# automl/RoBO

Hardware: NVIDIA H100
Metric: EI evals/sec (GP N=4096, D=16, fp64) (higher is better)
Workload: dtype f64

## Files before the change

### robo_b200/csrc/gpk_api.cu

```cuda
#include <algorithm>
#include <climits>
#include <cmath>
#include <cstdarg>
#include <cstdio>
#include <cstring>
#include <cstdlib>
#include <dlfcn.h>
#include <string>
#include <vector>

#include "gpk_gemm.cuh"
#include "gpk_kernels.cuh"
#include "gpk_diag16.cuh"
#include "gpk_ozaki.cuh"
#include "gpk_de.cuh"
#include "gpk_lbfgs.cuh"
#include "gpk_cmaes.cuh"
#include "gpk_direct.cuh"
#include "gpk_es.cuh"
#include "gpk_esmc.cuh"
#include "gpk_rs.cuh"
#include "gpk_hyper.cuh"
#include "gpk_blr.cuh"
#include "gpk_rf.cuh"
// ... 293 lines not shown
    cfg.dynamicSmemBytes = smem;
    cfg.stream = stream;
    cudaLaunchAttribute attr[1];
    attr[0].id = cudaLaunchAttributeClusterDimension;
    attr[0].val.clusterDim.x = (unsigned)cs;
    attr[0].val.clusterDim.y = 1;
    attr[0].val.clusterDim.z = 1;
    cfg.attrs = attr;
    cfg.numAttrs = cs > 1 ? 1 : 0;
    return cudaLaunchKernelEx(&cfg, kernel, KArgs(args)...);
}

int oz_max_clusters(gpk_handle* h, int cs, int* out) {
    if (h->oz_max_clusters[cs] == 0) {
        if (cs == 1) {
            h->oz_max_clusters[cs] = std::max(h->n_sm, 1);
        } else {
            cudaLaunchConfig_t cfg;
            memset(&cfg, 0, sizeof(cfg));
            cfg.gridDim = dim3((unsigned)cs);
            cfg.blockDim = dim3(OZ_THREADS);
            cfg.dynamicSmemBytes = OZ_SMEM;
            cudaLaunchAttribute attr[1];
            attr[0].id = cudaLaunchAttributeClusterDimension;
            attr[0].val.clusterDim.x = (unsigned)cs;
            attr[0].val.clusterDim.y = 1;
            attr[0].val.clusterDim.z = 1;
            cfg.attrs = attr;
            cfg.numAttrs = 1;
            int n = 0;
            CK(cudaOccupancyMaxActiveClusters(&n, gpk_oz_vargemm_kernel, &cfg));
            if (n < 1) { set_err(h, "no cluster of %d int8 contraction CTAs fits on this device", cs); return GPK_CUDA_ERROR; }
            h->oz_max_clusters[cs] = n;
        }
    }
    *out = h->oz_max_clusters[cs];
    return GPK_OK;
}

int launch_oz_contraction(gpk_handle* h, const CUtensorMap& mapP, const CUtensorMap& mapK, int nb, long rows_padded,
                          long NP, long rows, const int* eP, int eK, double* part_ssq, long ldpart) {
    OzArgs o;
    o.nb = nb; o.ncb = (int)(rows_padded / OZ_TN); o.NP = (int)NP; o.rows = (int)rows;
    const int cs = h->oz_cluster;
    o.group = (int)std::min<long>(512, std::max<long>(4, ((long)24 << 20) / ((long)OZ_TN * NP * OZ_S))) / cs * cs;
    o.eP = eP; o.eK = eK;
    o.part_ssq = part_ssq; o.ldpart = ldpart;
    const int persist = h->oz_persist == 3 ? (nb <= 32 ? 1 : 0) : h->oz_persist;
    const int tiles = o.nb * o.ncb;
    int grid = tiles;
    if (persist == 1) {
        int nclusters = 0, rc;
        if ((rc = oz_max_clusters(h, cs, &nclusters))) return rc;
        if (h->oz_grid > 0) nclusters = std::min(nclusters, h->oz_grid);
        grid = cs * std::min(tiles / cs, nclusters);
    }
    h->oz_last_variant = 1 + (persist == 1 ? 8 : 0) + (cs == 2 ? 16 : cs == 4 ? 32 : 0);
    CK(launch_oz(gpk_oz_vargemm_kernel, (unsigned)grid, cs, (size_t)OZ_SMEM, h->stream, mapP, mapK, o));
    CKL();
    return GPK_OK;
}

template <int EPI, int MI = 8>
int launch_gemm(gpk_handle* h, const CUtensorMap& mA, const CUtensorMap& mB, const GemmArgs& a, int njobs,
                cudaStream_t stream = nullptr) {
    static_assert(MI == 8 || (MI == 2 && EPI == EPI_STORE), "128-row tiles, or 32-row chain tiles that store");
    if (njobs <= 0) return GPK_OK;
    if (stream == nullptr) stream = h->stream;
    if constexpr (MI == 2) {
        CK(launch_pdl(gpk_gemm_nt_kernel, dim3(njobs), dim3(GEMM_THREADS), (size_t)GEMM_SMEM_CHAIN, stream, mA, mB, a));
        h->launches_total += 1;
        return GPK_OK;
    }
    gpk_gemm_ws_kernel<EPI><<<njobs, WS_THREADS, GEMM_SMEM_TMA, stream>>>(mA, mB, a);
    CKL();
    return GPK_OK;
}

int set_kernel_attrs(gpk_handle* h) {
    CK(cudaFuncSetAttribute(gpk_gemm_ws_kernel<EPI_STORE>, cudaFuncAttributeMaxDynamicSharedMemorySize, GEMM_SMEM_TMA));
    CK(cudaFuncSetAttribute(gpk_gemm_ws_kernel<EPI_COLREDUCE>, cudaFuncAttributeMaxDynamicSharedMemorySize, GEMM_SMEM_TMA));
    CK(cudaFuncSetAttribute(gpk_gemm_nt_kernel, cudaFuncAttributeMaxDynamicSharedMemorySize, GEMM_SMEM_CHAIN));
    CK(cudaFuncSetAttribute(gpk_oz_vargemm_kernel, cudaFuncAttributeMaxDynamicSharedMemorySize, OZ_SMEM));
    CK(cudaFuncSetAttribute(gpk_cov_oz_kernel<8>, cudaFuncAttributeMaxDynamicSharedMemorySize, (int)cov_oz_smem_bytes(GPK_MAX_TERMS, 8)));
    CK(cudaFuncSetAttribute(gpk_cov_oz_kernel<4>, cudaFuncAttributeMaxDynamicSharedMemorySize, (int)cov_oz_smem_bytes(GPK_MAX_TERMS, 4)));
    CK(cudaFuncSetAttribute(gpk_cov_oz_kernel<8, false>, cudaFuncAttributeMaxDynamicSharedMemorySize, (int)cov_oz_smem_bytes(GPK_MAX_TERMS, 8)));
    {
        cudaDeviceProp prop;
        CK(cudaGetDeviceProperties(&prop, h->device));
        h->n_sm = prop.multiProcessorCount;
    }
    CK(cudaFuncSetAttribute(gpk_cov_tma_kernel<8>, cudaFuncAttributeMaxDynamicSharedMemorySize, (int)cov_tma_smem_bytes(GPK_MAX_TERMS, 8)));
    CK(cudaFuncSetAttribute(gpk_cov_tma_kernel<4>, cudaFuncAttributeMaxDynamicSharedMemorySize, (int)cov_tma_smem_bytes(GPK_MAX_TERMS, 4)));
    CK(cudaFuncSetAttribute(gpk_potrf_diag_dmma_kernel, cudaFuncAttributeMaxDynamicSharedMemorySize, DIAG_SMEM));
    return GPK_OK;
}

struct Node { int lo, mid, hi, height; };

int build_nodes(int lo, int hi, std::vector<Node>& nodes) {
    if (hi - lo <= 1) return 0;
    int mid = lo + (hi - lo + 1) / 2;
    int hl = build_nodes(lo, mid, nodes);
    int hr = build_nodes(mid, hi, nodes);
    int ht = 1 + std::max(hl, hr);
    nodes.push_back({lo, mid, hi, ht});
    return ht;
}

int build_job_tables(gpk_handle* h) {
    const int nb = h->nb;
    if (h->jobs_nb == nb) return GPK_OK;
    std::vector<GemmJob> jobs;
    h->syrk_r.assign(nb, Range());
    for (int k = 0; k < nb; ++k) {
        h->syrk_r[k].off = (int)jobs.size();
        for (int j = k + 1; j < nb; ++j)
            for (int i = j; i <= nb; ++i)
                jobs.push_back({i * BM, j * BM, k * BM, (k + 1) * BM, i * BM, j * BM, 0, 0});
        h->syrk_r[k].cnt = (int)jobs.size() - h->syrk_r[k].off;
    }
    h->syrk2_r.assign(nb, Range());
    for (int k = 1; k < nb; k += 2) {
        h->syrk2_r[k].off = (int)jobs.size();
        for (int j = k + 2; j < nb; ++j)
            for (int i = j; i <= nb; ++i)
                jobs.push_back({i * BM, j * BM, (k - 1) * BM, (k + 1) * BM, i * BM, j * BM, 0, 0});
        h->syrk2_r[k].cnt = (int)jobs.size() - h->syrk2_r[k].off;
    }
    h->trsm32_r.assign(nb, Range());
    h->pu32_r.assign(nb, Range());
    for (int k = 0; k < nb; ++k) {
        h->trsm32_r[k].off = (int)jobs.size();
        for (int i = k + 1; i <= nb; ++i)
            for (int q = 0; q < 4; ++q) {
                if (i == nb && q > 0) break;
                jobs.push_back({i * BM + 32 * q, k * BM, k * BM, (k + 1) * BM, i * BM + 32 * q, k * BM, 0, 0});
            }
        h->trsm32_r[k].cnt = (int)jobs.size() - h->trsm32_r[k].off;
        h->pu32_r[k].off = (int)jobs.size();
        if (k + 1 < nb)
            for (int i = k + 1; i <= nb; ++i)
                for (int q = 0; q < 4; ++q) {
                    if (i == nb && q > 0) break;
                    jobs.push_back({i * BM + 32 * q, (k + 1) * BM, k * BM, (k + 1) * BM, i * BM + 32 * q, (k + 1) * BM, 0, 0});
                }
        h->pu32_r[k].cnt = (int)jobs.size() - h->pu32_r[k].off;
    }
    std::vector<Node> nodes;
    int hmax = build_nodes(0, nb, nodes);
    h->tri1_r.assign(hmax + 1, Range());
    h->tri2_r.assign(hmax + 1, Range());
    auto by_len = [](const GemmJob& a, const GemmJob& b) { return (a.k1 - a.k0) > (b.k1 - b.k0); };
    for (int ht = 1; ht <= hmax; ++ht) {
        size_t s1 = jobs.size();
        for (const Node& nd : nodes) {
            if (nd.height != ht) continue;
            for (int c = nd.lo; c < nd.mid; ++c)
                for (int i = nd.mid; i < nd.hi; ++i)
                    jobs.push_back({c * BM, i * BM, c * BM, nd.mid * BM, c * BM, i * BM, 0, 0});
        }
        std::stable_sort(jobs.begin() + s1, jobs.end(), by_len);
        h->tri1_r[ht].off = (int)s1;
        h->tri1_r[ht].cnt = (int)(jobs.size() - s1);
        size_t s2 = jobs.size();
        for (const Node& nd : nodes) {
            if (nd.height != ht) continue;
            for (int i = nd.mid; i < nd.hi; ++i)
                for (int c = nd.lo; c < nd.mid; ++c)
// ... 327 lines not shown

ScoreOut score_out(gpk_handle* h, int kind, double eta, double par, double* d_out, double* d_mu, double* d_var,
                   unsigned long long* d_nneg, long offset, long global_base) {
    ScoreOut o;
    o.base = global_base + offset;
    o.acq_kind = kind; o.eta = eta; o.par = par;
    o.out_mu = d_mu ? d_mu + offset : nullptr;
    o.out_var = d_var ? d_var + offset : nullptr;
    o.out_acq = d_out ? d_out + offset : nullptr;
    o.block_best = ptr<BestPair>(h->block_best);
    o.n_negative = d_nneg;
    return o;
}

int score_dev(gpk_handle* h, const double* dX, long m, int kind, double eta, double par, double* d_out,
              double* d_mu, double* d_var, BestPair* d_best, unsigned long long* d_nneg,
              long index_offset = 0, bool reset = true, long global_base = 0, Feeder* feeder = nullptr) {
    if (h->model != MODEL_GP)
        return surrogate_score(h, dX, m, kind, eta, par, d_out, d_mu, d_var, d_best, d_nneg, index_offset, reset,
                               global_base, feeder);
    int rc = build_linv(h);
    if (rc) return rc;
    const long NP = h->NP;
    const long cap = std::min<long>(chunk_rows(h), round_up(std::max<long>(m, 1), BM));
    if ((rc = ensure_score_scratch(h, cap))) return rc;
    bool use_oz = false;
    if (m >= 2048 && (rc = prepare_ozaki(h, &use_oz))) return rc;
    int oz_eK = 0;
    if (use_oz) {
        if ((rc = ensure(h, h->oz_Kq, (size_t)OZ_S * cap * NP))) return rc;
        if (h->overlap && (rc = ensure(h, h->oz_Kq2, (size_t)OZ_S * cap * NP))) return rc;
        if ((rc = make_oz_map(h, &h->mapOzK, h->oz_Kq.p, (long)OZ_S * cap, NP, OZ_TN))) return rc;
        if (h->overlap && (rc = make_oz_map(h, &h->mapOzK2, h->oz_Kq2.p, (long)OZ_S * cap, NP, OZ_TN))) return rc;
        if (h->overlap && (rc = ensure(h, h->oz_pmu2, (size_t)h->nb * cap * 8))) return rc;
        oz_eK = oz_exponent(h->spec.amp);
    }
    if (d_best == nullptr) d_best = ptr<BestPair>(h->best);
    if (d_nneg == nullptr) d_nneg = ptr<unsigned long long>(h->nneg);
    if (reset) {
        CK(cudaMemsetAsync(d_best, 0xFF, sizeof(BestPair), h->stream));
        CK(cudaMemsetAsync(d_nneg, 0, 8, h->stream));
    }
    CK(cudaEventRecord(h->ev[6], h->stream));
    const int nchunks = (int)((m + cap - 1) / cap);
    const bool pipelined = h->overlap && nchunks > 1;
    if (pipelined) {
        while ((int)h->ev_cov.size() < nchunks) {
            cudaEvent_t e1, e2;
            CK(cudaEventCreateWithFlags(&e1, cudaEventDisableTiming));
            CK(cudaEventCreateWithFlags(&e2, cudaEventDisableTiming));
            h->ev_cov.push_back(e1);
            h->ev_gemm.push_back(e2);
        }
    }
    while ((int)h->ev_g0.size() < nchunks) {
        cudaEvent_t e1, e2;
        CK(cudaEventCreate(&e1));
        CK(cudaEventCreate(&e2));
        h->ev_g0.push_back(e1);
        h->ev_g1.push_back(e2);
    }
    h->last_nchunks = nchunks;
    auto launch_cov = [&](int ci, cudaStream_t st, bool small) -> int {
        const long base = (long)ci * cap;
        const long mc = std::min(cap, m - base);
        const long mcp = round_up(mc, BM);
        const bool second = pipelined && (ci & 1);
        if (feeder) {
            int frc = feeder->ready(base, base + mc, st);
            if (frc) return frc;
        }
        const double* lo = h->has_bounds ? ptr<double>(h->lower) : nullptr;
        const double* up = h->has_bounds ? ptr<double>(h->upper) : nullptr;
        if (!use_oz)
            return launch_cov_tiles(h, st, ptr<double>(h->Xts), NP, h->n, dX + base * h->d, h->d, mc, mcp, lo, up,
                                    second ? ptr<double>(h->Kstar2) : ptr<double>(h->Kstar), NP, 0, small,
                                    ptr<double>(h->Xrow), nullptr, nullptr);
        CUtensorMap map;
        int mrc = make_cov_map(h, &map, h->Xts.p, h->spec.n_terms, NP);
        if (mrc) return mrc;
        int8_t* qdst = second ? ptr<int8_t>(h->oz_Kq2) : ptr<int8_t>(h->oz_Kq);
        double* pmu = second ? ptr<double>(h->oz_pmu2) : ptr<double>(h->part_mu);
        const int gx = (int)(NP / 128);
        if (small)
            gpk_cov_oz_kernel<4><<<(unsigned)(gx * (mcp / 16)), 256, cov_oz_smem_bytes(h->spec.n_terms, 4), st>>>(
                map, h->spec, h->n, dX + base * h->d, h->d, mc, lo, up, ptr<double>(h->alpha), oz_eK, qdst, NP, cap * NP, pmu, cap, gx,
                nullptr);
        else
            gpk_cov_oz_kernel<8><<<(unsigned)(gx * (mcp / 32)), 256, cov_oz_smem_bytes(h->spec.n_terms, 8), st>>>(
                map, h->spec, h->n, dX + base * h->d, h->d, mc, lo, up, ptr<double>(h->alpha), oz_eK, qdst, NP, cap * NP, pmu, cap, gx,
                nullptr);
        CKL();
        return GPK_OK;
    };
    if (pipelined) {
        CK(cudaEventRecord(h->ev_order, h->stream));
        CK(cudaStreamWaitEvent(h->side_stream, h->ev_order, 0));
        if ((rc = launch_cov(0, h->side_stream, false))) return rc;
        CK(cudaEventRecord(h->ev_cov[0], h->side_stream));
    }
    for (int ci = 0; ci < nchunks; ++ci) {
        const long base = (long)ci * cap;
        const long mc = std::min(cap, m - base);
        const long mcp = round_up(mc, BM);
        const bool last = ci == nchunks - 1;
        if (last) CK(cudaEventRecord(h->ev[8], h->stream));
        if (pipelined) {
            CK(cudaStreamWaitEvent(h->stream, h->ev_cov[ci], 0));
            if (ci + 1 < nchunks) {
                if (ci >= 1) CK(cudaStreamWaitEvent(h->side_stream, h->ev_gemm[ci - 1], 0));
                if ((rc = launch_cov(ci + 1, h->side_stream, true))) return rc;
                CK(cudaEventRecord(h->ev_cov[ci + 1], h->side_stream));
            }
        } else {
            if ((rc = launch_cov(ci, h->stream, false))) return rc;
        }
        const bool second = pipelined && (ci & 1);
        GemmArgs a;
        memset(&a, 0, sizeof(a));
        a.A = ptr<double>(h->P); a.lda = NP;
        a.B = second ? ptr<double>(h->Kstar2) : ptr<double>(h->Kstar); a.ldb = NP;
        a.alpha = 1.0;
        a.job_mode = JOBS_VARIANCE;
        a.nb = h->nb; a.mcb = (int)(mcp / BN);
        a.z = ptr<double>(h->Kbuf) + NP * NP;
        a.part_mu = ptr<double>(h->part_mu);
        a.part_ssq = ptr<double>(h->part_ssq);
        a.ldpart = cap;
        if (last) CK(cudaEventRecord(h->ev[10], h->stream));
        CK(cudaEventRecord(h->ev_g0[ci], h->stream));
        if (use_oz) {
            if ((rc = launch_oz_contraction(h, h->mapOzP, second ? h->mapOzK2 : h->mapOzK, h->nb, mcp, NP, cap,
                                            ptr<int>(h->oz_eP), oz_eK, a.part_ssq, a.ldpart)))
                return rc;
            h->oz_launches += 1;
        } else if ((rc = launch_gemm<EPI_COLREDUCE>(h, h->mapP, second ? h->mapKs2 : h->mapKs, a, h->nb * a.mcb))) return rc;
        CK(cudaEventRecord(h->ev_g1[ci], h->stream));
        if (last) CK(cudaEventRecord(h->ev[11], h->stream));
        if (pipelined && !use_oz) CK(cudaEventRecord(h->ev_gemm[ci], h->stream));
        h->launches_var += 1;
        h->last_chunk_rows = mcp;
        FinishArgs f;
        memset(&f, 0, sizeof(f));
        f.part_mu = ptr<double>(h->part_mu); f.part_ssq = ptr<double>(h->part_ssq);
        f.ldpart = cap; f.nparts = h->nb; f.m = mc;
        f.kss = h->spec.amp; f.mean = h->mean;
        f.factor = h->spec.factor;
        f.cand = dX + base * h->d; f.cand_dc = h->d;
        f.lo = h->has_bounds ? ptr<double>(h->lower) : nullptr;
        f.up = h->has_bounds ? ptr<double>(h->upper) : nullptr;
        f.norm_out = h->norm_out; f.y_mean = h->y_mean; f.y_std = h->y_std;
        f.o = score_out(h, kind, eta, par, d_out, d_mu, d_var, d_nneg, index_offset + base, global_base);
        if (use_oz && second) f.part_mu = ptr<double>(h->oz_pmu2);
        const int fb = (int)((mc + 255) / 256);
        gpk_finish_kernel<<<fb, 256, 0, h->stream>>>(f);
        CKL();
        if (kind != GPK_ACQ_NONE) {
            gpk_argmax_final_kernel<<<1, 256, 0, h->stream>>>(ptr<BestPair>(h->block_best), fb, d_best);
            CKL();
        }
        if (pipelined && use_oz) CK(cudaEventRecord(h->ev_gemm[ci], h->stream));
        if (last) CK(cudaEventRecord(h->ev[12], h->stream));
    }
    CK(cudaEventRecord(h->ev[7], h->stream));
    h->score_timed = true;
    return GPK_OK;
}

struct EsLayout {
    size_t logP, lmb, dMu, dSig, Hs, W, lo, up, zb, total;
    EsLayout(int nb, int np_, int d) {
        const size_t T = (size_t)nb * (nb + 1) / 2;
        logP = 0; lmb = logP + nb; dMu = lmb + nb; dSig = dMu + (size_t)nb * nb; Hs = dSig + nb * T; W = Hs + nb * T;
        lo = W + np_; up = lo + d; zb = up + d; total = zb + (size_t)nb * d;
    }
};

struct McLayout {
    size_t Mb, Vb, W, lmb, zb, F, total;
    McLayout(int nb, int np_, int d, int nf) {
        Mb = 0; Vb = Mb + nb; W = Vb + (size_t)nb * nb; lmb = W + np_; zb = lmb + nb; F = zb + (size_t)nb * d;
        total = F + (size_t)nb * nf;
    }
};

enum { ES_KIND_NONE = 0, ES_KIND_EP = 1, ES_KIND_MC = 2 };

int predict_mean_dev(gpk_handle* h, const double* dX, long m, double* d_mu) {
    if (!h->mean_only)
        return score_dev(h, dX, m, GPK_ACQ_NONE, 0.0, 0.0, nullptr, d_mu, nullptr, nullptr, nullptr);
    int rc;
    if ((rc = build_linv(h))) return rc;
    if ((rc = ensure_alpha(h))) return rc;
    const long NP = h->NP;
    const long cap = std::min<long>(chunk_rows(h), round_up(m, BM));
    if ((rc = ensure(h, h->part_mu, (size_t)h->nb * cap * 8))) return rc;
    CUtensorMap map;
    if ((rc = make_cov_map(h, &map, h->Xts.p, h->spec.n_terms, NP))) return rc;
    const double* lo = h->has_bounds ? ptr<double>(h->lower) : nullptr;
    const double* up = h->has_bounds ? ptr<double>(h->upper) : nullptr;
    const int gx = (int)(NP / 128);
    for (long base = 0; base < m; base += cap) {
        const long mc = std::min(cap, m - base);
        const long mcp = round_up(mc, BM);
        gpk_cov_oz_kernel<8, false><<<(unsigned)(gx * (mcp / 32)), 256, cov_oz_smem_bytes(h->spec.n_terms, 8), h->stream>>>(
            map, h->spec, h->n, dX + base * h->d, h->d, mc, lo, up, ptr<double>(h->alpha), 0, nullptr, NP, 0,
            ptr<double>(h->part_mu), cap, gx, ptr<double>(h->Xrow));
        CKL();
        gpk_mu_parts_finish_kernel<<<(unsigned)((mc + 255) / 256), 256, 0, h->stream>>>(
            ptr<double>(h->part_mu), cap, h->nb, mc, h->mean, h->norm_out, h->y_mean, h->y_std, d_mu + base);
        CKL();
    }
    return GPK_OK;
}

const long ES_CH = 16384;

int es_reserve(gpk_handle* h) {
    return ensure(h, h->es_work, (size_t)ES_CH * (h->es_nb + 1) * 8);
}

int es_moments_pass(gpk_handle* h, const double* X, long rows) {
    const int nb = h->es_nb, d = h->d;
    const double* zs = h->es_kind == ES_KIND_MC ? ptr<double>(h->mc_state) + McLayout(nb, h->es_np, d, h->es_nf).zb
                                                : ptr<double>(h->es_state) + EsLayout(nb, h->es_np, d).zb;
    double* var = ptr<double>(h->es_work);
    double* sig = var + ES_CH;
    const double* lo = h->has_bounds ? ptr<double>(h->lower) : nullptr;
    const double* up = h->has_bounds ? ptr<double>(h->upper) : nullptr;
    const double out_scale = h->norm_out ? h->y_std * h->y_std : 1.0;
    int rc;
    if ((rc = score_dev(h, X, rows, GPK_ACQ_NONE, 0.0, 0.0, nullptr, nullptr, var, nullptr, nullptr))) return rc;
    gpk_es_sigma_kernel<<<(unsigned)rows, GPK_ES_THREADS, 0, h->stream>>>(h->spec, X, rows, d, lo, up,
                                                                          ptr<double>(h->Xrow), h->n,
                                                                          ptr<double>(h->es_U), zs, nb,
                                                                          out_scale, sig);
    CKL();
    return GPK_OK;
}

int es_dh_dev(gpk_handle* h, const double* Xm, const double* Xb, long m, double* d_out) {
    const int nb = h->es_nb, d = h->d;
    EsLayout L(nb, h->es_np, d);
    const double* st = ptr<double>(h->es_state);
    const long CH = ES_CH;
    int rc;
    if ((rc = es_reserve(h))) return rc;
    const double* var = ptr<double>(h->es_work);
    const double* sig = var + CH;
    for (long c0 = 0; c0 < m; c0 += CH) {
        const long rows = std::min(CH, m - c0);
        if ((rc = es_moments_pass(h, Xm + c0 * d, rows))) return rc;
        gpk_es_dh_kernel<<<(unsigned)rows, GPK_ES_THREADS, 0, h->stream>>>(
            Xb + c0 * d, rows, d, st + L.lo, st + L.up, var, sig, nb, h->es_np, h->es_sn2, h->es_H, st + L.logP,
            st + L.lmb, st + L.dMu, st + L.dSig, st + L.Hs, st + L.W, d_out + c0);
        CKL();
    }
    return GPK_OK;
}

int es_ready(gpk_handle* h, gpk_handle* report, const char* who, int kind = ES_KIND_EP) {
    gpk_handle* r = report ? report : h;
    const char* upd = kind == ES_KIND_MC ? "gpk_esmc_update" : "gpk_es_update";
    if (gp_refusal(h)) { set_err(r, "%s: %s", who, gp_refusal(h)); return GPK_BAD_ARG; }
    if (h->es_linv_serial < 0) { set_err(r, "%s: call %s first", who, upd); return GPK_BAD_ARG; }
    if (!h->linv_ready || h->es_linv_serial != h->linv_serial) {
        set_err(r, "%s: the model changed since %s", who, upd);
        return GPK_BAD_ARG;
    }
    if (kind != ES_KIND_NONE && h->es_kind != kind) {
        set_err(r, "%s: the current update is %s, not %s", who,
                h->es_kind == ES_KIND_MC ? "gpk_esmc_update" : "gpk_es_update", upd);
        return GPK_BAD_ARG;
    }
    return GPK_OK;
}

int es_build_u(gpk_handle* h, const double* zb, int nb, double* zs) {
    const int d = h->d, n = h->n, NP = h->NP;
    const size_t D = (size_t)nb;
    cudaStream_t s = h->stream;
    int rc;
    if ((rc = ensure(h, h->tmp1, D * d * 8))) return rc;
    CK(cudaMemcpyAsync(h->tmp1.p, zb, D * d * 8, cudaMemcpyHostToDevice, s));
    const double* lo = h->has_bounds ? ptr<double>(h->lower) : nullptr;
    const double* up = h->has_bounds ? ptr<double>(h->upper) : nullptr;
    gpk_es_scale_kernel<<<(unsigned)((D * d + 255) / 256), 256, 0, s>>>(ptr<double>(h->tmp1), nb, d, lo, up, zs);
    CKL();
// ... 2425 lines not shown
```

### robo_b200/csrc/gpk_ozaki.cuh

```cuda
#pragma once
#include "gpk_gemm.cuh"

constexpr int OZ_S = 7;
constexpr int OZ_PAIRS = OZ_S * (OZ_S + 1) / 2;
constexpr int OZ_TM = 128, OZ_TN = 32;
constexpr int OZ_KB = 64;
constexpr int OZ_UK = 32;
constexpr int OZ_NSTG = 3;
constexpr int OZ_A_SLICE = OZ_TM * OZ_KB, OZ_B_SLICE = OZ_TN * OZ_KB;
constexpr int OZ_STAGE = OZ_S * (OZ_A_SLICE + OZ_B_SLICE);
constexpr int OZ_THREADS = 384;
constexpr int OZ_SMEM = OZ_NSTG * OZ_STAGE + 1024 + 256 + 2 * 8 * OZ_TN * 8;
constexpr int OZ_MAX_EXP = 7;

__host__ __device__ inline int oz_exponent(double amax) {
    if (!(amax > 0.0)) return 0;
    int ex;
    const double m = frexp(amax, &ex);
    return ex + 1 + (m * 128.0 >= 127.49 ? 1 : 0);
}
__device__ __forceinline__ unsigned long long oz_digits(double v) {
    const long long X = __double2ll_rn(v * 72057594037927936.0);
    return (unsigned long long)(X + 0x0080808080808080LL) ^ 0x0080808080808080ULL;
}
// ... 151 lines not shown
                                    bar_full + 8 * s);
                    }
                }
            }
        }
        if (cs > 1) oz_cluster_sync();
        return;
    }
    asm volatile("setmaxnreg.inc.sync.aligned.u32 232;" ::: "memory");
    const int c = wg - 1, cw = (tid - 128) >> 5;
    const int r0 = c * 64 + (cw & 3) * 16 + (lane >> 2);
    int it = 0, tl = 0;
    for (int t = cid; t < total; t += ncl, ++tl) {
        int ib, cbc;
        oz_tile_of(t, g.nb, ncbc, gc, ib, cbc);
        const int cb = cbc * (int)cs + (int)rank;
        const int nkb = (ib + 1) * OZ_TM / OZ_KB;
        uint32_t acc[OZ_S][16];
#pragma unroll
        for (int l = 0; l < OZ_S; ++l)
#pragma unroll
            for (int e = 0; e < 16; ++e) acc[l][e] = 0u;
        uint32_t fa[2][2][4];
        for (int kb = 0; kb < nkb; kb += 2) {
#pragma unroll
            for (int h = 0; h < 2; ++h, ++it) {
                const int s = it % OZ_NSTG;
                oz_mbar_wait(bar_full + 8 * s, (uint32_t)((it / OZ_NSTG) & 1));
                const uint32_t st = base + s * OZ_STAGE;
#pragma unroll
                for (int a = 0; a < OZ_S; ++a) {
                    uint32_t (&f)[2][4] = fa[(h * OZ_S + a) & 1];
                    oz_lda_frag(f, st + a * OZ_A_SLICE, c * 64 + (cw & 3) * 16, lane);
                    wgmma_arrive();
#pragma unroll
                    for (int tk = 0; tk < OZ_S - a; ++tk)
#pragma unroll
                        for (int k = 0; k < OZ_KB / OZ_UK; ++k)
                            oz_wgmma_rs(acc[a + tk], f[k], oz_desc(st + OZ_S * OZ_A_SLICE + tk * OZ_B_SLICE + k * OZ_UK));
                    wgmma_commit();
                    wgmma_wait_one();
                    if (a == 0 && (h == 1 || kb > 0) && (uint32_t)(tid & 127) < cs)
                        oz_release_stage(bar_empty + 8 * ((it + OZ_NSTG - 1) % OZ_NSTG), cs, (uint32_t)(tid & 127));
                }
            }
        }
        wgmma_wait_all();
#pragma unroll
        for (int l = 0; l < OZ_S; ++l) oz_wgmma_fence(acc[l]);
        if ((uint32_t)(tid & 127) < cs) oz_release_stage(bar_empty + 8 * ((it + OZ_NSTG - 1) % OZ_NSTG), cs, (uint32_t)(tid & 127));
        const double rs0 = ldexp(1.0, g.eP[ib * OZ_TM + r0] + g.eK), rs1 = ldexp(1.0, g.eP[ib * OZ_TM + r0 + 8] + g.eK);
        double col[8];
#pragma unroll
        for (int j = 0; j < 8; ++j) col[j] = 0.0;
#pragma unroll
        for (int e = 0; e < 16; ++e) {
            double v = 0.0;
#pragma unroll
            for (int lvl = OZ_S - 1; lvl >= 0; --lvl) v = fma(oz_i2d(acc[lvl][e]), ldexp(1.0, -8 * (lvl + 2)), v);
            const double x = v * (((e >> 1) & 1) ? rs1 : rs0);
            col[2 * (e >> 2) + (e & 1)] += x * x;
        }
#pragma unroll
        for (int j = 0; j < 8; ++j)
#pragma unroll
            for (int o = 4; o < 32; o <<= 1) col[j] += __shfl_xor_sync(0xffffffffu, col[j], o);
        const uint32_t redt = red + (uint32_t)((tl & 1) * 8 * OZ_TN * 8);
        if (lane < 4) {
#pragma unroll
            for (int j = 0; j < 8; ++j) sts64(redt + (uint32_t)((cw * OZ_TN + 8 * (j >> 1) + 2 * lane + (j & 1)) * 8), col[j]);
        }
        named_bar_sync(1, 256);
        const int et = tid - 128;
        if (et < OZ_TN) {
            double s2 = 0.0;
#pragma unroll
            for (int w8 = 0; w8 < 8; ++w8) s2 += lds64(redt + (uint32_t)((w8 * OZ_TN + et) * 8));
            g.part_ssq[(long)ib * g.ldpart + cb * OZ_TN + et] = s2;
        }
    }
    if (cs > 1) oz_cluster_sync();
}

template <int CC, bool DIGITS = true>
__global__ void __launch_bounds__(256, CC == 8 ? 2 : 4)
gpk_cov_oz_kernel(const __grid_constant__ CUtensorMap mapX, const KSpec ks, int n,
                  const double* __restrict__ cand, int dc, long m,
                  const double* __restrict__ lower, const double* __restrict__ upper,
                  const double* __restrict__ alpha, int eK, int8_t* __restrict__ Kq, long ldq, long slice_stride,
                  double* __restrict__ part_mu, long ldpart, int gx, const double* __restrict__ Xenv)
{
    constexpr int TC = 4 * CC;
    extern __shared__ unsigned char cov_raw[];
    const int tid = threadIdx.x;
    const long w = blockIdx.x;
    const int bx = (int)(w % gx);
    const long c0 = (w / gx) * TC;
    const int nt = ks.n_terms;
    const uint32_t base = (cov_smem_u32(cov_raw) + 127u) & ~127u;
    const uint32_t xs = base;
    const uint32_t scb = xs + (uint32_t)nt * 1024u;
    const uint32_t bar = scb + (uint32_t)(TC * nt) * 8u;
    const uint32_t mred = bar + 8u;
    if (tid == 0) {
        asm volatile("mbarrier.init.shared::cta.b64 [%0], 1;" :: "r"(bar) : "memory");
        asm volatile("fence.mbarrier_init.release.cluster;" ::: "memory");
        asm volatile("fence.proxy.async.shared::cta;" ::: "memory");
        asm volatile("mbarrier.arrive.expect_tx.shared::cta.b64 _, [%0], %1;" :: "r"(bar), "r"((uint32_t)nt * 1024u) : "memory");
        asm volatile("cp.async.bulk.tensor.2d.shared::cluster.global.mbarrier::complete_tx::bytes [%0], [%1, {%3, %4}], [%2];"
                     :: "r"(xs), "l"((uint64_t)&mapX), "r"(bar), "r"(bx * 128), "r"(0) : "memory");
    }
    const int jp = tid & 63, cgp = tid >> 6, lane = tid & 31;
    const double sc = ldexp(1.0, -eK);
    for (int e = tid; e < TC * nt; e += 256) {
        const int c = e / nt, t = e - c * nt;
        const long ci = c0 + c;
        double v = 0.0;
        if (ci < m) {
            const int a = ks.axis[t];
            v = cand[ci * dc + a];
            if (lower != nullptr) v = (v - lower[a]) / (upper[a] - lower[a]);
            v *= ks.scale[t];
        }
        asm volatile("st.shared.f64 [%0], %1;" :: "r"(scb + (uint32_t)e * 8u), "d"(v) : "memory");
    }
    __syncthreads();
    {
        uint32_t ok = 0;
        while (!ok)
            asm volatile("{\n\t.reg .pred p;\n\tmbarrier.try_wait.parity.shared::cta.b64 p, [%1], 0;\n\tselp.u32 %0, 1, 0, p;\n\t}"
                         : "=r"(ok) : "r"(bar) : "memory");
    }
    double q[CC][2], pr[CC][2];
#pragma unroll
    for (int c = 0; c < CC; ++c) { q[c][0] = q[c][1] = 0.0; pr[c][0] = pr[c][1] = 1.0; }
    const uint32_t xrow = xs + (uint32_t)jp * 16u;
    const uint32_t srow = scb + (uint32_t)(cgp * CC * nt) * 8u;
    for (int t = 0; t < nt; ++t) {
        double x0, x1;
        asm volatile("ld.shared.v2.f64 {%0, %1}, [%2];" : "=d"(x0), "=d"(x1) : "r"(xrow + (uint32_t)t * 1024u));
#pragma unroll
        for (int c = 0; c < CC; ++c) {
            double sv;
            asm volatile("ld.shared.f64 %0, [%1];" : "=d"(sv) : "r"(srow + (uint32_t)(c * nt + t) * 8u));
            const double d0 = sv - x0, d1 = sv - x1;
            q[c][0] = fma(d0, d0, q[c][0]);
            q[c][1] = fma(d1, d1, q[c][1]);
        }
        if (ks.last[t]) {
#pragma unroll
            for (int c = 0; c < CC; ++c) {
                pr[c][0] *= gpk_radial_q(ks.family, q[c][0]);
                pr[c][1] *= gpk_radial_q(ks.family, q[c][1]);
                q[c][0] = q[c][1] = 0.0;
            }
        }
    }
    const int j0 = bx * 128 + 2 * jp;
    const bool v0 = j0 < n, v1 = j0 + 1 < n;
    const double a0 = v0 ? alpha[j0] : 0.0, a1 = v1 ? alpha[j0 + 1] : 0.0;
#pragma unroll
    for (int c = 0; c < CC; ++c) {
        const long ci = c0 + cgp * CC + c;
        const bool cv = ci < m;
        double k0 = (cv && v0) ? ks.amp * pr[c][0] : 0.0;
        double k1 = (cv && v1) ? ks.amp * pr[c][1] : 0.0;
        if (!DIGITS && ks.factor.kind != GPK_FACTOR_NONE && cv) {
            const double zc = gpk_factor_coord(ks.factor, cand + ci * dc, lower, upper);
            if (v0) k0 *= gpk_factor_value(ks.factor, zc, Xenv[(long)j0 * dc + ks.factor.axis]);
            if (v1) k1 *= gpk_factor_value(ks.factor, zc, Xenv[(long)(j0 + 1) * dc + ks.factor.axis]);
        }
        if (DIGITS) {
            const unsigned long long y0 = oz_digits(k0 * sc), y1 = oz_digits(k1 * sc);
            int8_t* dst = Kq + ci * ldq + j0;
#pragma unroll
            for (int s2 = 0; s2 < OZ_S; ++s2)
                *reinterpret_cast<uint16_t*>(dst + (long)s2 * slice_stride) = (uint16_t)(oz_digit_of(y0, s2) | (oz_digit_of(y1, s2) << 8));
        }
        double pm = fma(k0, a0, k1 * a1);
#pragma unroll
        for (int off = 16; off > 0; off >>= 1) pm += __shfl_xor_sync(0xffffffffu, pm, off);
        if (lane == 0) asm volatile("st.shared.f64 [%0], %1;" :: "r"(mred + (uint32_t)(((tid >> 5) * CC + c) * 8)), "d"(pm) : "memory");
    }
    __syncthreads();
    if (tid < TC) {
        const int g = tid / CC, c = tid - g * CC;
        double lo2, hi2;
        asm volatile("ld.shared.f64 %0, [%1];" : "=d"(lo2) : "r"(mred + (uint32_t)(((2 * g) * CC + c) * 8)));
        asm volatile("ld.shared.f64 %0, [%1];" : "=d"(hi2) : "r"(mred + (uint32_t)(((2 * g + 1) * CC + c) * 8)));
        part_mu[(long)bx * ldpart + c0 + tid] = lo2 + hi2;
    }
}
inline size_t cov_oz_smem_bytes(int n_terms, int cc) { return (size_t)n_terms * 1024 + (size_t)4 * cc * n_terms * 8 + 8 + 8 * cc * 8 + 128; }

__device__ __forceinline__ void oz_wgmma_n128(uint32_t (&d)[64], uint64_t a_desc, uint64_t b_desc, uint32_t accumulate) {
    asm volatile("{\n\t.reg .pred p;\n\tsetp.ne.b32 p, %66, 0;\n\t"
                 "wgmma.mma_async.sync.aligned.m64n128k32.s32.s8.s8 "
                 "{%0, %1, %2, %3, %4, %5, %6, %7, %8, %9, %10, %11, %12, %13, %14, %15, %16, %17, %18, %19, %20, %21, %22, %23, %24, %25, %26, %27, %28, %29, %30, %31, %32, %33, %34, %35, %36, %37, %38, %39, %40, %41, %42, %43, %44, %45, %46, %47, %48, %49, %50, %51, %52, %53, %54, %55, %56, %57, %58, %59, %60, %61, %62, %63}, %64, %65, p;\n\t}"
                 : "+r"(d[0]), "+r"(d[1]), "+r"(d[2]), "+r"(d[3]), "+r"(d[4]), "+r"(d[5]), "+r"(d[6]), "+r"(d[7]),
                   "+r"(d[8]), "+r"(d[9]), "+r"(d[10]), "+r"(d[11]), "+r"(d[12]), "+r"(d[13]), "+r"(d[14]), "+r"(d[15]),
                   "+r"(d[16]), "+r"(d[17]), "+r"(d[18]), "+r"(d[19]), "+r"(d[20]), "+r"(d[21]), "+r"(d[22]), "+r"(d[23]),
                   "+r"(d[24]), "+r"(d[25]), "+r"(d[26]), "+r"(d[27]), "+r"(d[28]), "+r"(d[29]), "+r"(d[30]), "+r"(d[31]),
                   "+r"(d[32]), "+r"(d[33]), "+r"(d[34]), "+r"(d[35]), "+r"(d[36]), "+r"(d[37]), "+r"(d[38]), "+r"(d[39]),
                   "+r"(d[40]), "+r"(d[41]), "+r"(d[42]), "+r"(d[43]), "+r"(d[44]), "+r"(d[45]), "+r"(d[46]), "+r"(d[47]),
                   "+r"(d[48]), "+r"(d[49]), "+r"(d[50]), "+r"(d[51]), "+r"(d[52]), "+r"(d[53]), "+r"(d[54]), "+r"(d[55]),
                   "+r"(d[56]), "+r"(d[57]), "+r"(d[58]), "+r"(d[59]), "+r"(d[60]), "+r"(d[61]), "+r"(d[62]), "+r"(d[63])
                 : "l"(a_desc), "l"(b_desc), "r"(accumulate));
}
__device__ __forceinline__ void oz_wgmma_fence64(uint32_t (&d)[64]) {
#pragma unroll
    for (int i = 0; i < 64; i += 16) oz_wgmma_fence(*reinterpret_cast<uint32_t(*)[16]>(d + i));
}
__global__ void __launch_bounds__(256, 1) gpk_peak_i8_kernel(int iters, int random_operands, unsigned* sink)
{
    extern __shared__ unsigned char pk_raw[];
    const uint32_t base = (smem_u32(pk_raw) + 1023u) & ~1023u;
    const int tid = threadIdx.x, wg = tid >> 7;
    for (int e = tid; e < 4096; e += 256) {
        uint32_t w = 0x01010101u * (e & 3);
        if (random_operands) { w = (uint32_t)e * 2654435761u + blockIdx.x * 40503u; w ^= w >> 15; w *= 2246822519u; w ^= w >> 13; }
        asm volatile("st.shared.u32 [%0], %1;" :: "r"(base + 4u * e), "r"(w) : "memory");
    }
    fence_proxy_async();
    __syncthreads();
    uint32_t d[64];
#pragma unroll
    for (int i = 0; i < 64; ++i) d[i] = 0u;
    const uint32_t a0 = base + wg * 64 * 64;
    const uint64_t da0 = oz_desc(a0), da1 = oz_desc(a0 + 32), db0 = oz_desc(base + 8192), db1 = oz_desc(base + 8192 + 32);
    for (int i = 0; i < iters; i += 8) {
        oz_wgmma_fence64(d);
        wgmma_arrive();
#pragma unroll
        for (int j = 0; j < 8; ++j) {
            oz_wgmma_n128(d, da0, db0, 1u);
            oz_wgmma_n128(d, da1, db1, 1u);
        }
        wgmma_commit();
        asm volatile("wgmma.wait_group.sync.aligned 1;" ::: "memory");
        oz_wgmma_fence64(d);
    }
    wgmma_wait_all();
    oz_wgmma_fence64(d);
    uint32_t x = 0;
#pragma unroll
    for (int i = 0; i < 64; ++i) x ^= d[i];
    if (x == 0x9e3779b9u) sink[0] = x;
}
```

Measured before the change: 2.634 million.

## Stage Ozaki digit tiles in shared memory and reduce-scatter the mean shuffles

The covariance Ozaki kernel now writes its int8 digit slices into a shared-memory staging tile and then copies them out with coalesced 16-byte global stores, instead of scattered 2-byte global writes per thread. The per-candidate warp reductions for the mean are replaced by a reduce-scatter across the eight candidates, which cuts the number of shuffles. The small CC=4 variant is removed, so only CC=8 remains, and the launch bounds change to 3 blocks per SM. This costs extra shared memory (7*32*128 bytes for staging) and an additional pass after the sync, and small batches lose their specialised variant.

```diff
diff --git a/robo_b200/csrc/gpk_api.cu b/robo_b200/csrc/gpk_api.cu
--- a/robo_b200/csrc/gpk_api.cu
+++ b/robo_b200/csrc/gpk_api.cu
@@ -399,9 +399,8 @@
     CK(cudaFuncSetAttribute(gpk_gemm_ws_kernel<EPI_COLREDUCE>, cudaFuncAttributeMaxDynamicSharedMemorySize, GEMM_SMEM_TMA));
     CK(cudaFuncSetAttribute(gpk_gemm_nt_kernel, cudaFuncAttributeMaxDynamicSharedMemorySize, GEMM_SMEM_CHAIN));
     CK(cudaFuncSetAttribute(gpk_oz_vargemm_kernel, cudaFuncAttributeMaxDynamicSharedMemorySize, OZ_SMEM));
-    CK(cudaFuncSetAttribute(gpk_cov_oz_kernel<8>, cudaFuncAttributeMaxDynamicSharedMemorySize, (int)cov_oz_smem_bytes(GPK_MAX_TERMS, 8)));
-    CK(cudaFuncSetAttribute(gpk_cov_oz_kernel<4>, cudaFuncAttributeMaxDynamicSharedMemorySize, (int)cov_oz_smem_bytes(GPK_MAX_TERMS, 4)));
-    CK(cudaFuncSetAttribute(gpk_cov_oz_kernel<8, false>, cudaFuncAttributeMaxDynamicSharedMemorySize, (int)cov_oz_smem_bytes(GPK_MAX_TERMS, 8)));
+    CK(cudaFuncSetAttribute(gpk_cov_oz_kernel<true>, cudaFuncAttributeMaxDynamicSharedMemorySize, (int)cov_oz_smem_bytes(GPK_MAX_TERMS, true)));
+    CK(cudaFuncSetAttribute(gpk_cov_oz_kernel<false>, cudaFuncAttributeMaxDynamicSharedMemorySize, (int)cov_oz_smem_bytes(GPK_MAX_TERMS, false)));
     {
         cudaDeviceProp prop;
         CK(cudaGetDeviceProperties(&prop, h->device));
@@ -895,14 +894,9 @@
         int8_t* qdst = second ? ptr<int8_t>(h->oz_Kq2) : ptr<int8_t>(h->oz_Kq);
         double* pmu = second ? ptr<double>(h->oz_pmu2) : ptr<double>(h->part_mu);
         const int gx = (int)(NP / 128);
-        if (small)
-            gpk_cov_oz_kernel<4><<<(unsigned)(gx * (mcp / 16)), 256, cov_oz_smem_bytes(h->spec.n_terms, 4), st>>>(
-                map, h->spec, h->n, dX + base * h->d, h->d, mc, lo, up, ptr<double>(h->alpha), oz_eK, qdst, NP, cap * NP, pmu, cap, gx,
-                nullptr);
-        else
-            gpk_cov_oz_kernel<8><<<(unsigned)(gx * (mcp / 32)), 256, cov_oz_smem_bytes(h->spec.n_terms, 8), st>>>(
-                map, h->spec, h->n, dX + base * h->d, h->d, mc, lo, up, ptr<double>(h->alpha), oz_eK, qdst, NP, cap * NP, pmu, cap, gx,
-                nullptr);
+        gpk_cov_oz_kernel<true><<<(unsigned)(gx * (mcp / COV_OZ_TC)), 256, cov_oz_smem_bytes(h->spec.n_terms, true), st>>>(
+            map, h->spec, h->n, dX + base * h->d, h->d, mc, lo, up, ptr<double>(h->alpha), oz_eK, qdst, NP, cap * NP, pmu, cap, gx,
+            nullptr);
         CKL();
         return GPK_OK;
     };
@@ -1016,7 +1010,7 @@
     for (long base = 0; base < m; base += cap) {
         const long mc = std::min(cap, m - base);
         const long mcp = round_up(mc, BM);
-        gpk_cov_oz_kernel<8, false><<<(unsigned)(gx * (mcp / 32)), 256, cov_oz_smem_bytes(h->spec.n_terms, 8), h->stream>>>(
+        gpk_cov_oz_kernel<false><<<(unsigned)(gx * (mcp / COV_OZ_TC)), 256, cov_oz_smem_bytes(h->spec.n_terms, false), h->stream>>>(
             map, h->spec, h->n, dX + base * h->d, h->d, mc, lo, up, ptr<double>(h->alpha), 0, nullptr, NP, 0,
             ptr<double>(h->part_mu), cap, gx, ptr<double>(h->Xrow));
         CKL();
diff --git a/robo_b200/csrc/gpk_ozaki.cuh b/robo_b200/csrc/gpk_ozaki.cuh
--- a/robo_b200/csrc/gpk_ozaki.cuh
+++ b/robo_b200/csrc/gpk_ozaki.cuh
@@ -257,15 +257,19 @@
     if (cs > 1) oz_cluster_sync();
 }
 
-template <int CC, bool DIGITS = true>
-__global__ void __launch_bounds__(256, CC == 8 ? 2 : 4)
+constexpr int COV_OZ_CC = 8;
+constexpr int COV_OZ_TC = 4 * COV_OZ_CC;
+
+template <bool DIGITS>
+__global__ void __launch_bounds__(256, 3)
 gpk_cov_oz_kernel(const __grid_constant__ CUtensorMap mapX, const KSpec ks, int n,
                   const double* __restrict__ cand, int dc, long m,
                   const double* __restrict__ lower, const double* __restrict__ upper,
                   const double* __restrict__ alpha, int eK, int8_t* __restrict__ Kq, long ldq, long slice_stride,
                   double* __restrict__ part_mu, long ldpart, int gx, const double* __restrict__ Xenv)
 {
-    constexpr int TC = 4 * CC;
+    constexpr int CC = COV_OZ_CC, TC = COV_OZ_TC;
+    static_assert(CC == 8, "the mean share's reduce-scatter takes three halving steps to one candidate per lane");
     extern __shared__ unsigned char cov_raw[];
     const int tid = threadIdx.x;
     const long w = blockIdx.x;
@@ -276,7 +280,8 @@
     const uint32_t xs = base;
     const uint32_t scb = xs + (uint32_t)nt * 1024u;
     const uint32_t bar = scb + (uint32_t)(TC * nt) * 8u;
-    const uint32_t mred = bar + 8u;
+    const uint32_t mred = bar + 16u;
+    const uint32_t stg = mred + 8u * CC * 8u;
     if (tid == 0) {
         asm volatile("mbarrier.init.shared::cta.b64 [%0], 1;" :: "r"(bar) : "memory");
         asm volatile("fence.mbarrier_init.release.cluster;" ::: "memory");
@@ -334,6 +339,7 @@
     const int j0 = bx * 128 + 2 * jp;
     const bool v0 = j0 < n, v1 = j0 + 1 < n;
     const double a0 = v0 ? alpha[j0] : 0.0, a1 = v1 ? alpha[j0 + 1] : 0.0;
+    double pm[CC];
 #pragma unroll
     for (int c = 0; c < CC; ++c) {
         const long ci = c0 + cgp * CC + c;
@@ -347,16 +353,30 @@
         }
         if (DIGITS) {
             const unsigned long long y0 = oz_digits(k0 * sc), y1 = oz_digits(k1 * sc);
-            int8_t* dst = Kq + ci * ldq + j0;
+            const uint32_t dst = stg + (uint32_t)((cgp * CC + c) * 128 + 2 * jp);
 #pragma unroll
             for (int s2 = 0; s2 < OZ_S; ++s2)
-                *reinterpret_cast<uint16_t*>(dst + (long)s2 * slice_stride) = (uint16_t)(oz_digit_of(y0, s2) | (oz_digit_of(y1, s2) << 8));
-        }
-        double pm = fma(k0, a0, k1 * a1);
-#pragma unroll
-        for (int off = 16; off > 0; off >>= 1) pm += __shfl_xor_sync(0xffffffffu, pm, off);
-        if (lane == 0) asm volatile("st.shared.f64 [%0], %1;" :: "r"(mred + (uint32_t)(((tid >> 5) * CC + c) * 8)), "d"(pm) : "memory");
-    }
+                asm volatile("st.shared.u16 [%0], %1;"
+                             :: "r"(dst + (uint32_t)(s2 * TC * 128)),
+                                "h"((unsigned short)(oz_digit_of(y0, s2) | (oz_digit_of(y1, s2) << 8))) : "memory");
+        }
+        pm[c] = fma(k0, a0, k1 * a1);
+    }
+#pragma unroll
+    for (int h = 0; h < 3; ++h) {
+        const int off = 16 >> h, half = CC >> (h + 1);
+        const bool up = (lane & off) != 0;
+#pragma unroll
+        for (int i = 0; i < half; ++i) {
+            const double keep = up ? pm[i + half] : pm[i];
+            const double send = up ? pm[i] : pm[i + half];
+            pm[i] = keep + __shfl_xor_sync(0xffffffffu, send, off);
+        }
+    }
+    pm[0] += __shfl_xor_sync(0xffffffffu, pm[0], 2);
+    pm[0] += __shfl_xor_sync(0xffffffffu, pm[0], 1);
+    const int lc = ((lane >> 4) & 1) * 4 + ((lane >> 3) & 1) * 2 + ((lane >> 2) & 1);
+    if ((lane & 3) == 0) asm volatile("st.shared.f64 [%0], %1;" :: "r"(mred + (uint32_t)(((tid >> 5) * CC + lc) * 8)), "d"(pm[0]) : "memory");
     __syncthreads();
     if (tid < TC) {
         const int g = tid / CC, c = tid - g * CC;
@@ -365,8 +385,22 @@
         asm volatile("ld.shared.f64 %0, [%1];" : "=d"(hi2) : "r"(mred + (uint32_t)(((2 * g + 1) * CC + c) * 8)));
         part_mu[(long)bx * ldpart + c0 + tid] = lo2 + hi2;
     }
-}
-inline size_t cov_oz_smem_bytes(int n_terms, int cc) { return (size_t)n_terms * 1024 + (size_t)4 * cc * n_terms * 8 + 8 + 8 * cc * 8 + 128; }
+    if (DIGITS) {
+        for (int e = tid; e < OZ_S * TC * 8; e += 256) {
+            const int s2 = e / (TC * 8), r = e - s2 * (TC * 8), cl = r >> 3, k = r & 7;
+            uint32_t d0, d1, d2, d3;
+            asm volatile("ld.shared.v4.u32 {%0, %1, %2, %3}, [%4];"
+                         : "=r"(d0), "=r"(d1), "=r"(d2), "=r"(d3) : "r"(stg + (uint32_t)e * 16u));
+            int8_t* dst = Kq + (long)s2 * slice_stride + (c0 + cl) * ldq + bx * 128 + 16 * k;
+            asm volatile("st.global.v4.u32 [%0], {%1, %2, %3, %4};"
+                         :: "l"(dst), "r"(d0), "r"(d1), "r"(d2), "r"(d3) : "memory");
+        }
+    }
+}
+inline size_t cov_oz_smem_bytes(int n_terms, bool digits) {
+    return (size_t)n_terms * 1024 + (size_t)COV_OZ_TC * n_terms * 8 + 16 + 8 * COV_OZ_CC * 8
+           + (digits ? (size_t)OZ_S * COV_OZ_TC * 128 : 0) + 128;
+}
 
 __device__ __forceinline__ void oz_wgmma_n128(uint32_t (&d)[64], uint64_t a_desc, uint64_t b_desc, uint32_t accumulate) {
     asm volatile("{\n\t.reg .pred p;\n\tsetp.ne.b32 p, %66, 0;\n\t"
```

Result: no change. 2.646 million (median of 6 runs) (+0.4%).
